# guanlongzhao/fac-via-ppg

Hardware: AMD Instinct MI355X
Metric: 22.05 kHz audio samples/sec end-to-end PPG→wav; real-time factor at batch=1 (higher is better)
Workload: dtype f32

## Files before the change

### fac-via-ppg_amd/csrc/facppg_wg.hip

```cpp
#include <algorithm>
#include <cmath>
#include <cstdlib>
#include <cstring>
#include <new>
#include <type_traits>
#include <vector>

#include "facppg_gemm.h"
#include "facppg_wg_internal.h"

namespace facppg {

thread_local char g_err[512] = "";
void set_error(const char* fmt, ...) {
  va_list ap;
  va_start(ap, fmt);
  vsnprintf(g_err, sizeof(g_err), fmt, ap);
  va_end(ap);
}

namespace {

constexpr int TN = 64;
constexpr int HALO = 128;
// ... 216 lines not shown
      const int mid = (lo + hi + 1) >> 1;
      if (off[mid] <= g) lo = mid; else hi = mid - 1;
    }
    const int q = 4 * (g - off[lo]);
    e = make_int4(lo, q, t_valid[lo] - q, 0);
  }
  table[g] = e;
}

struct WnArgs {
  const float* h_in;
  float* h_out;
  const float* spect;
  float* skip;
  const float4* w1;
  const float* b1;
  const float4* w2;
  const float* b2;
  const int* t_valid;
  int T, hop8, Lp, Lr, dil, first;
  float* save_ts;
  const float* melp;
  const float4* wc;
  int P, Tr, Tqp, ntq, nt, nch, ngc, kc, xcd_map;
  int hop, ksize;
  int flat_cols;
  const int4* groups;
  const float* xa;
  const float* we;
  const float* endb;
  int nconv;
  const float4* seed;
  int seed_nt;
};

typedef float f4u __attribute__((ext_vector_type(4), aligned(4)));

template <int NRB>
__device__ __forceinline__ void load_a(float4 (&a)[4], const float4* __restrict__ p, int rb_stride, int g) {
#pragma unroll
  for (int rb = 0; rb < NRB; ++rb) a[rb] = p[rb * rb_stride + g * 64];
}

template <int NCB, bool K4 = false>
__device__ __forceinline__ void load_b(float (&bv)[4][NCB], const float* lb, int g) {
  if constexpr (K4) {
#pragma unroll
    for (int cb = 0; cb < NCB; ++cb) {
      const float4 v = *reinterpret_cast<const float4*>(lb + ((2 * g) * (32 * NCB) + 32 * cb) * 4);
      bv[0][cb] = v.x; bv[1][cb] = v.y; bv[2][cb] = v.z; bv[3][cb] = v.w;
    }
  } else {
#pragma unroll
    for (int s = 0; s < 4; ++s)
#pragma unroll
      for (int cb = 0; cb < NCB; ++cb) bv[s][cb] = lb[(8 * g + s) * (32 * NCB) + 32 * cb];
  }
}

__device__ __forceinline__ int k4_index(int k, int col, int tnt) { return ((k >> 2) * tnt + col) * 4 + (k & 3); }

template <int NRB, int NCB>
__device__ __forceinline__ void mfma_group(f32x16 (&acc)[4][NCB], const float4 (&a)[4], const float (&bv)[4][NCB]) {
#pragma unroll
  for (int s = 0; s < 4; ++s) {
#pragma unroll
// ... 370 lines not shown
        } else {
          const float vv[4] = {v.x, v.y, v.z, v.w};
          for (int k = 0; k < nv; ++k) gbase[o + k] = vv[k] + (add ? rbase[o + k] : 0.0f);
        }
      }
    }
    return;
  }
#pragma unroll
  for (int rb = 0; rb < NRB2; ++rb) {
    const bool is_res = !LAST && rb < 2;
    const int chb = w * 64 + (rb & 1) * 32 + 4 * kh;
#pragma unroll
    for (int cb = 0; cb < NCB; ++cb) {
      const int col = cb * 32 + li;
      if (col < nvalid) {
#pragma unroll
        for (int r = 0; r < 16; ++r) {
          const int ch = chb + 8 * (r >> 2) + (r & 3);
          if (is_res) {
            const size_t o = ((size_t)b * C + ch) * p.Lp + in_off + col;
            p.h_out[o] = acc[rb][cb][r];
          } else {
            const size_t o = ((size_t)b * C + ch) * p.Lr + sk_off + col;
            p.skip[o] = (p.first ? 0.0f : p.skip[o]) + acc[rb][cb][r];
          }
        }
      }
    }
  }
}

#ifdef FACPPG_WN8_PROF
__device__ unsigned long long g_wn8_prof[12];
#define WN8_STAMP_DECL long long wn8_t = clock64()
#define WN8_STAMP(i)                                                                           \
  do {                                                                                         \
    const long long now__ = clock64();                                                         \
    if (blockIdx.x == 0 && threadIdx.x == 0) { atomicAdd(&g_wn8_prof[i], (unsigned long long)(now__ - wn8_t)); if ((i) == 5) atomicAdd(&g_wn8_prof[6], 1ull); } \
    wn8_t = now__;                                                                             \
  } while (0)
#else
#define WN8_STAMP_DECL
#define WN8_STAMP(i)
#endif

typedef float f32x4s __attribute__((ext_vector_type(4)));
#define FACPPG_AS1 __attribute__((address_space(1)))
typedef float f32x4s __attribute__((ext_vector_type(4)));
__device__ __forceinline__ float4 gld(const float4* q) {
  const f32x4s v = *(const FACPPG_AS1 f32x4s*)q;
  return make_float4(v.x, v.y, v.z, v.w);
}
__device__ __forceinline__ f4u gld(const f4u* q) { return *(const FACPPG_AS1 f4u*)q; }
__device__ __forceinline__ float gld(const float* q) { return *(const FACPPG_AS1 float*)q; }
__device__ __forceinline__ void store_f4(float* g, const float4 v) {
  const f32x4s x = {v.x, v.y, v.z, v.w};
  *(FACPPG_AS1 f32x4s*)g = x;
}
__device__ __forceinline__ void store_f1(float* g, const float v) { *(__attribute__((address_space(1))) float*)g = v; }

template <bool LAST, int NCB, bool EF, bool SEED = false>
__device__ __forceinline__ void wn_layer8_tile(const WnArgs& p, const int lin, float* __restrict__ smem) {
  static_assert(!SEED || NCB == 1, "seeded tiles: 32 frames");
  constexpr int TNt = 32 * NCB;
  WN8_STAMP_DECL;
  const int tid = threadIdx.x, lane = tid & 63, w8 = tid >> 6, wq = w8 >> 1, sub = w8 & 1;
  const int li = lane & 31, kh = lane >> 5;
  const int chb = wq * 64 + sub * 32;
  int b, nvalid, ph, in_off, sk_off, tap0, tap1, tap2, lane_q;
  int tile;
  {
    if (p.xcd_map == 1) { const int r = lin >> 3; ph = (r / p.nt) * 8 + (lin & 7); tile = r % p.nt; }
    else { ph = lin / p.nt; tile = lin % p.nt; }
    if (ph >= p.P) return;
    int qcol;
    if (p.groups) {
      const int4 e = p.groups[tile * (TNt / 4) + lane % (TNt / 4)];
      if (__builtin_amdgcn_readfirstlane(e.z) <= 0) return;
      b = e.x; qcol = e.y; nvalid = e.z;
    } else if (p.flat_cols > 0) {
      const int c0 = tile * TNt + (lane % (TNt / 4)) * 4;
      const int cl = min(c0, p.flat_cols - 4);
      b = cl / p.T; qcol = cl - b * p.T; nvalid = p.flat_cols - c0;
    } else {
      b = tile / p.ntq;
      const int q0 = (tile % p.ntq) * TNt, Tb = p.t_valid ? p.t_valid[b] : p.T;
      if (q0 >= Tb) return;
      qcol = q0 + (lane % (TNt / 4)) * 4; nvalid = Tb - qcol;
    }
    in_off = ph * p.Tqp + HQ + qcol;
    sk_off = ph * p.Tr + qcol;
    lane_q = HQ + qcol;
    {
      const int pm = ph - p.dil, qm = pm >= 0 ? pm / p.P : -((p.P - 1 - pm) / p.P);
      const int pq = ph + p.dil, qp = pq / p.P;
      tap0 = (pm - qm * p.P) * p.Tqp + qm;
      tap1 = ph * p.Tqp;
      tap2 = (pq - qp * p.P) * p.Tqp + qp;
// ... 174 lines not shown
      f32x4 tot = {0.f, 0.f, 0.f, 0.f};
#pragma unroll
      for (int sl = 0; sl < 8; ++sl) {
        const float av[8] = {a0[sl].x, a0[sl].y, a0[sl].z, a0[sl].w, a1[sl].x, a1[sl].y, a1[sl].z, a1[sl].w};
        f32x4 e = {0.f, 0.f, 0.f, 0.f};
#pragma unroll
        for (int g = 0; g < 8; ++g) e = mfma16x16x4(av[g], gb[(8 * sl + g) * TNt * 4], e);
        if (sl == 0) tot = e;
        else { tot[0] += e[0]; tot[1] += e[1]; tot[2] += e[2]; tot[3] += e[3]; }
      }
      if (kq < 2) {
        float* endl = smem + C * TNt + (4 * kq) * TNt + 16 * w8 + pl;
#pragma unroll
        for (int r = 0; r < 4; ++r) endl[r * TNt] = tot[r];
      }
    }
  }
  __syncthreads();
  WN8_STAMP(4);
  if constexpr (EF) {
    const int row = w8 * RPL4 + srow4;
    if (row < 8 && nvalid > 0) {
      float4 v4 = *reinterpret_cast<const float4*>(smem + C * TNt + row * TNt + scol4);
      if constexpr (ESPLIT) {
#pragma unroll
        for (int sl = 1; sl < 8; ++sl) {
          const float4 x = *reinterpret_cast<const float4*>(smem + C * TNt + (sl * 8 + row) * TNt + scol4);
          v4.x += x.x; v4.y += x.y; v4.z += x.z; v4.w += x.w;
        }
      }
      float* g = p.skip + ((size_t)b * 8 + row) * p.Lr + sk_off;
      const float bias = p.endb[row];
      const float vv[4] = {v4.x, v4.y, v4.z, v4.w};
      if (nvalid >= 4) {
        float4 x = make_float4(bias, bias, bias, bias);
        if (!p.first) x = *reinterpret_cast<const float4*>(g);
        store_f4(g, make_float4(x.x + vv[0], x.y + vv[1], x.z + vv[2], x.w + vv[3]));
      } else {
        for (int k = 0; k < nvalid; ++k) store_f1(g + k, (p.first ? bias : g[k]) + vv[k]);
      }
    }
  }
  float* slab = smem + w8 * (32 * TNt);
#pragma unroll
  for (int half = 0; half < NRB2; ++half) {
    const bool is_res = EF || (!LAST && half == 0);
#pragma unroll
    for (int cb = 0; cb < NCB; ++cb)
#pragma unroll
      for (int r = 0; r < 16; ++r) slab[(8 * (r >> 2) + (r & 3) + 4 * kh) * TNt + cb * 32 + li] = acc[half][cb][r];
    const int nv = nvalid;
    if (nv <= 0) continue;
    float* gbase = is_res ? p.h_out + (size_t)b * C * p.Lp + in_off : p.skip + (size_t)b * C * p.Lr + sk_off;
    const float* rbase = is_res ? p.h_in + (size_t)b * C * p.Lp + in_off : gbase;
    const int pitch = is_res ? p.Lp : p.Lr;
    const bool add = is_res || !p.first;
#pragma unroll
    for (int i = 0; i < 32 / RPL4; ++i) {
      const int row = i * RPL4 + srow4;
      const size_t o = (size_t)(chb + row) * pitch;
      float4 v = *reinterpret_cast<const float4*>(slab + row * TNt + scol4);
      if (nv >= 4) {
        if (add) {
          float4 x;
          if (HPRE && is_res) x = hpre[i];
          else x = gld(reinterpret_cast<const float4*>(rbase + o));
          v.x += x.x; v.y += x.y; v.z += x.z; v.w += x.w;
        }
        store_f4(gbase + o, v);
      } else {
        const float vv[4] = {v.x, v.y, v.z, v.w};
        for (int k = 0; k < nv; ++k) store_f1(gbase + o + k, vv[k] + (add ? gld(rbase + o + k) : 0.0f));
      }
    }
  }
// ... 144 lines not shown
#pragma unroll
            for (int cb = 0; cb < NCB; ++cb) acc[rb][cb] = mfma32x32x2(av, bq[s4][cb], acc[rb][cb]);
          }
      }
    }
#pragma unroll
    for (int cb = 0; cb < NCB; ++cb) {
      const int tile = p.tile0 + blk * NCB + cb;
      if (tile >= p.seed_nt) continue;
      float4* dst = p.seeds + (((((size_t)l * p.P + ph) * p.seed_nt + tile) * 8 + w8) * 8) * 64 + lane;
#pragma unroll
      for (int rb = 0; rb < 2; ++rb)
#pragma unroll
        for (int q = 0; q < 4; ++q) {
          const f32x4s x = {acc[rb][cb][4 * q + 0], acc[rb][cb][4 * q + 1], acc[rb][cb][4 * q + 2], acc[rb][cb][4 * q + 3]};
          if constexpr (NT) __builtin_nontemporal_store(x, (FACPPG_AS1 f32x4s*)(dst + (rb * 4 + q) * 64));
          else *(FACPPG_AS1 f32x4s*)(dst + (rb * 4 + q) * 64) = x;
        }
    }
  }
  __syncthreads();
  if (p.counter) {
    if (tid == 0) reinterpret_cast<int*>(smem)[0] = (int)gridDim.x + atomicAdd(p.counter, 1);
    __syncthreads();
    lin = reinterpret_cast<const int*>(smem)[0];
    __syncthreads();
  } else lin += (int)gridDim.x;
  }
}

constexpr int TN16 = 16;

template <bool LAST, bool EF>
__device__ __forceinline__ void wn_layer16_tile(const WnArgs& p, const int ph, const int b, const int q0, float* __restrict__ smem) {
  const int tid = threadIdx.x, lane = tid & 63, w8 = tid >> 6;
  const int pl = lane & 15, kq = lane >> 4;
  const int chb = w8 * 32;
  const int nvalid = (p.t_valid ? p.t_valid[b] : p.T) - q0;
  if (nvalid <= 0) return;
  const int in_off = ph * p.Tqp + HQ + q0, sk_off = ph * p.Tr + q0;
  int tapo[3];
#pragma unroll
  for (int tp = 0; tp < 3; ++tp) {
    const int pp = ph + (tp - 1) * p.dil;
    const int qsh = pp >= 0 ? pp / p.P : -((p.P - 1 - pp) / p.P);
    tapo[tp] = (pp - qsh * p.P) * p.Tqp + HQ + q0 + qsh;
  }
  f32x4 acc[4];
  const float4* wave_a = p.w1 + (w8 * 4) * 64 + lane;
  const float4* wave_c = p.wc + (size_t)ph * (p.ngc / 2) * 2048 + (w8 * 4) * 64 + lane;
  const int nch = pm_chunks(p, ph), ncc = nch - p.nconv, NGC16 = ncc * 4;
  const int srow = tid >> 3, scol = (tid & 7) * 2;
  const bool folded_first = EF && p.nconv == 1;
  const float* hb = (folded_first ? p.xa + (size_t)b * 8 * p.Lp : p.h_in + (size_t)b * C * p.Lp) + scol;
  const float* sb = p.melp + (size_t)b * NMEL * p.Tqp + HQ + q0 + scol;
  typedef float f2u __attribute__((ext_vector_type(2), aligned(4)));
  float2 stg;
  auto stage_load = [&](int c) __attribute__((always_inline)) {
    const bool conv = c >= ncc;
    const int cc = c - ncc;
    const int r = min(c * 64 + srow, p.kc - 1);
    const int j = r / NMEL, m = r - j * NMEL;
    const int tp = folded_first ? min(srow >> 3, 2) : cc >> 2;
    const int chn = folded_first ? (srow & 7) : (cc & 3) * 64 + srow;
    const float* src = conv ? hb + (size_t)chn * p.Lp + (tp == 0 ? tapo[0] : tp == 1 ? tapo[1] : tapo[2])
                            : sb + m * p.Tqp - j;
    const f2u v = *reinterpret_cast<const f2u*>(src);
    stg = make_float2(v.x, v.y);
  };
  const int sw_r = srow & 15, sw_base = (((srow >> 4) * 4 + 2 * (sw_r & 1) + ((sw_r >> 2) & 1)) * TN16) * 4 + 2 * (sw_r >> 3) + ((sw_r >> 1) & 1);
  auto stage_write = [&](int buf) __attribute__((always_inline)) {
    float* dst = smem + buf * (KCH * TN16) + sw_base + scol * 4;
    dst[0] = stg.x; dst[4] = stg.y;
  };
  auto load_a = [&](float4 (&a)[4], int gg) __attribute__((always_inline)) {
    const float4* src = gg < NGC16 ? wave_c + (size_t)gg * 2048 : wave_a + (size_t)(gg - NGC16) * 2048;
#pragma unroll
    for (int rbl = 0; rbl < 4; ++rbl) a[rbl] = src[rbl * 64];
  };
  constexpr int RING = 4;
  float4 ar[RING][4];
  stage_load(0);
#pragma unroll
  for (int i = 0; i < RING - 1; ++i) load_a(ar[i], i);
#pragma unroll
  for (int rbl = 0; rbl < 4; ++rbl) {
    const float4 bv = *reinterpret_cast<const float4*>(p.b1 + (rbl >> 1) * C + chb + (rbl & 1) * 16 + 4 * kq);
    acc[rbl][0] = bv.x; acc[rbl][1] = bv.y; acc[rbl][2] = bv.z; acc[rbl][3] = bv.w;
  }
  stage_write(0);
  __syncthreads();
  for (int c = 0; c < nch; ++c) {
    stage_load(c + 1 < nch ? c + 1 : c);
    const float* lb = smem + (c & 1) * (KCH * TN16) + (kq * TN16 + pl) * 4;
#pragma unroll
    for (int g = 0; g < 4; ++g) {
      load_a(ar[(g + RING - 1) % RING], c * 4 + g + RING - 1);
      __builtin_amdgcn_sched_barrier(0);
      const float4 b4 = *reinterpret_cast<const float4*>(lb + g * (4 * TN16 * 4));
      const float bq[4] = {b4.x, b4.y, b4.z, b4.w};
#pragma unroll
      for (int s = 0; s < 4; ++s)
#pragma unroll
        for (int rbl = 0; rbl < 4; ++rbl) {
          const float4& a4 = ar[g % RING][rbl];
          acc[rbl] = mfma16x16x4(s == 0 ? a4.x : s == 1 ? a4.y : s == 2 ? a4.z : a4.w, bq[s], acc[rbl]);
        }
    }
    stage_write((c + 1) & 1);
    __syncthreads();
  }
#pragma unroll
  for (int rbl = 0; rbl < 2; ++rbl)
#pragma unroll
    for (int r = 0; r < 4; ++r)
      smem[(((2 * w8 + rbl) * 4 + 2 * (r & 1) + (kq & 1)) * TN16 + pl) * 4 + 2 * (kq >> 1) + ((r >> 1) & 1)] = gate_tanh_sigmoid(acc[rbl][r], acc[rbl + 2][r]);
  __syncthreads();
  constexpr int NB2 = EF ? (LAST ? 0 : 2) : LAST ? 2 : 4;
  constexpr bool ROWS256 = LAST || EF;
  float4 hpre[2];
  if constexpr (!LAST) {
    if (nvalid - (lane & 3) * 4 >= 4) {
#pragma unroll
      for (int it = 0; it < 2; ++it)
        hpre[it] = *reinterpret_cast<const float4*>(p.h_in + ((size_t)b * C + chb + it * 16 + (lane >> 2)) * p.Lp + in_off + (lane & 3) * 4);
    }
  }
#pragma unroll
  for (int rbl = 0; rbl < NB2; ++rbl) {
    const float4 bv = *reinterpret_cast<const float4*>(p.b2 + (ROWS256 ? 0 : (rbl >> 1) * C) + chb + (rbl & 1) * 16 + 4 * kq);
    acc[rbl][0] = bv.x; acc[rbl][1] = bv.y; acc[rbl][2] = bv.z; acc[rbl][3] = bv.w;
  }
  if constexpr (NB2 > 0) {
    const float4* ap2 = p.w2 + (w8 * NB2) * 64 + lane;
    const float* lb = smem + (kq * TN16 + pl) * 4;
    auto load_a2 = [&](float4 (&a)[4], int g) __attribute__((always_inline)) {
#pragma unroll
      for (int rbl = 0; rbl < NB2; ++rbl) a[rbl] = ap2[(size_t)g * (NB2 * 8 * 64) + rbl * 64];
    };
#pragma unroll
    for (int i = 0; i < RING - 1; ++i) load_a2(ar[i], i);
    for (int c = 0; c < C / 64; ++c) {
#pragma unroll
      for (int g = 0; g < 4; ++g) {
        load_a2(ar[(g + RING - 1) % RING], c * 4 + g + RING - 1);
        __builtin_amdgcn_sched_barrier(0);
        const float4 b4 = *reinterpret_cast<const float4*>(lb + (4 * c + g) * (4 * TN16 * 4));
        const float bq[4] = {b4.x, b4.y, b4.z, b4.w};
#pragma unroll
        for (int s = 0; s < 4; ++s)
#pragma unroll
          for (int rbl = 0; rbl < NB2; ++rbl) {
            const float4& a4 = ar[g % RING][rbl];
            acc[rbl] = mfma16x16x4(s == 0 ? a4.x : s == 1 ? a4.y : s == 2 ? a4.z : a4.w, bq[s], acc[rbl]);
          }
      }
    }
  }
  if constexpr (EF) {
    const float4* wimg = reinterpret_cast<const float4*>(p.we) + w8 * 128 + lane * 2;
    const float4 a0 = wimg[0], a1 = wimg[1];
    const float av[8] = {a0.x, a0.y, a0.z, a0.w, a1.x, a1.y, a1.z, a1.w};
    f32x4 e = {0.f, 0.f, 0.f, 0.f};
#pragma unroll
    for (int g = 0; g < 8; ++g)
      e = mfma16x16x4(av[g], smem[(((2 * w8 + (g >> 2)) * 4 + 2 * (kq & 1) + (g & 1)) * TN16 + pl) * 4 + 2 * ((g & 3) >> 1) + (kq >> 1)], e);
    if (kq < 2) {
      float* part = smem + C * TN16 + (w8 * 8 + 4 * kq) * TN16 + pl;
#pragma unroll
      for (int r = 0; r < 4; ++r) part[r * TN16] = e[r];
    }
  }
  __syncthreads();
  if constexpr (EF) {
    if (tid < 32) {
      const int row = tid >> 2, c4 = (tid & 3) * 4, nv = nvalid - c4;
      if (nv > 0) {
        const float* part = smem + C * TN16 + row * TN16 + c4;
        float4 t = *reinterpret_cast<const float4*>(part);
#pragma unroll
        for (int sl = 1; sl < 8; ++sl) {
          const float4 x = *reinterpret_cast<const float4*>(part + sl * 8 * TN16);
          t.x += x.x; t.y += x.y; t.z += x.z; t.w += x.w;
        }
        float* g = p.skip + ((size_t)b * 8 + row) * p.Lr + sk_off + c4;
        const float bias = p.endb[row];
        const float vv[4] = {t.x, t.y, t.z, t.w};
        if (nv >= 4) {
          float4 x = make_float4(bias, bias, bias, bias);
          if (!p.first) x = *reinterpret_cast<const float4*>(g);
          *reinterpret_cast<float4*>(g) = make_float4(x.x + vv[0], x.y + vv[1], x.z + vv[2], x.w + vv[3]);
        } else {
          for (int k = 0; k < nv; ++k) g[k] = (p.first ? bias : g[k]) + vv[k];
        }
      }
    }
  }
  float* slab = smem + w8 * (32 * TN16);
  const int erow = lane >> 2, ecol = (lane & 3) * 4;
#pragma unroll
  for (int half = 0; half < NB2 / 2; ++half) {
    const bool is_res = EF || (!LAST && half == 0);
#pragma unroll
    for (int rbl = 0; rbl < 2; ++rbl)
#pragma unroll
      for (int r = 0; r < 4; ++r) slab[(16 * rbl + 4 * kq + r) * TN16 + pl] = acc[half * 2 + rbl][r];
    const int nv = nvalid - ecol;
    if (nv <= 0) continue;
    float* gbase = is_res ? p.h_out + (size_t)b * C * p.Lp + in_off + ecol : p.skip + (size_t)b * C * p.Lr + sk_off + ecol;
    const float* rbase = is_res ? p.h_in + (size_t)b * C * p.Lp + in_off + ecol : gbase;
    const int pitch = is_res ? p.Lp : p.Lr;
    const bool add = is_res || !p.first;
#pragma unroll
    for (int it = 0; it < 2; ++it) {
      const int row = it * 16 + erow;
      const size_t o = (size_t)(chb + row) * pitch;
      float4 v = *reinterpret_cast<const float4*>(slab + row * TN16 + ecol);
      if (nv >= 4) {
        if (add) {
          float4 x;
          if (!LAST && is_res) x = hpre[it];
          else x = *reinterpret_cast<const float4*>(rbase + o);
          v.x += x.x; v.y += x.y; v.z += x.z; v.w += x.w;
        }
        *reinterpret_cast<float4*>(gbase + o) = v;
      } else {
        const float vv[4] = {v.x, v.y, v.z, v.w};
        for (int k = 0; k < nv; ++k) gbase[o + k] = vv[k] + (add ? rbase[o + k] : 0.0f);
      }
    }
  }
}

template <bool LAST, bool EF = false>
__global__ __launch_bounds__(512, 4) void k_wn_layer16(WnArgs p) {
  extern __shared__ __attribute__((aligned(16))) float smem[];
  int ph, tile;
  {
    const int lin = blockIdx.x;
    if (p.xcd_map == 1) { const int r = lin >> 3; ph = (r / p.nt) * 8 + (lin & 7); tile = r % p.nt; }
    else { ph = lin / p.nt; tile = lin % p.nt; }
    if (ph >= p.P) return;
  }
  wn_layer16_tile<LAST, EF>(p, ph, tile / p.ntq, (tile % p.ntq) * TN16, smem);
}

template <bool LAST>
__global__ __launch_bounds__(512, 4) void k_wn_layer_mixed(WnArgs p32, WnArgs p16, int n32) {
  extern __shared__ __attribute__((aligned(16))) float smem[];
  const int lin = (int)blockIdx.x, nt = p32.nt;
  int ph, tile;
  if (p32.xcd_map == 1) { const int r = lin >> 3; ph = (r / nt) * 8 + (lin & 7); tile = r % nt; }
  else { ph = lin / nt; tile = lin % nt; }
  if (ph >= p32.P) return;
  if (tile < n32) wn_layer8_tile<LAST, 1, true, true>(p32, lin, smem);
  else wn_layer16_tile<LAST, true>(p16, ph, 0, 32 * n32 + (tile - n32) * TN16, smem);
}

constexpr int UP_QB = 32;
constexpr int UP_MAXJ = 8;

__global__ __launch_bounds__(256) void k_upsample(const float* __restrict__ mel, const float* __restrict__ W,
                                                  const float* __restrict__ bias, float* __restrict__ spect,
                                                  const int* __restrict__ t_valid, int T, int n_mel, int hop,
                                                  int ksize, int Lr, int n_limit) {
  extern __shared__ float smel[];
  const int b = blockIdx.z, m = blockIdx.y, q0 = blockIdx.x * UP_QB;
  const int Tb = t_valid ? t_valid[b] : T;
  if (q0 >= Tb) return;
  const int nj = (ksize + hop - 1) / hop;
  const int SW = UP_QB + UP_MAXJ;
  for (int i = threadIdx.x; i < n_mel * SW; i += blockDim.x) {
    const int mp = i / SW, tt = i % SW;
    const int t = q0 - (UP_MAXJ - 1) + tt;
    smel[i] = (t >= 0 && t < Tb && tt < UP_QB + UP_MAXJ - 1) ? mel[((size_t)b * n_mel + mp) * T + t] : 0.0f;
  }
  __syncthreads();
  for (int pp = threadIdx.x; pp < hop; pp += blockDim.x) {
    float acc[UP_QB];
    const float bv = bias[m];
#pragma unroll
    for (int q = 0; q < UP_QB; ++q) acc[q] = bv;
    for (int j = 0; j < nj; ++j) {
      const int k = pp + j * hop;
      if (k < ksize) {
        for (int mp = 0; mp < n_mel; ++mp) {
          const float wv = W[((size_t)mp * n_mel + m) * ksize + k];
          const float* sm = smel + mp * SW + (UP_MAXJ - 1) - j;
#pragma unroll
// ... 736 lines not shown
PmLayout pm_layout(const facppg_wg_config& c, int B, int T) {
  PmLayout w;
  w.P = c.hop_length / 8;
  w.L = T * w.P;
  w.La = round_up(w.L, TN);
  w.Tr = round_up(T, TN);
  w.Tqp = HQ + w.Tr + HQ;
  size_t off = 0;
  auto take = [&](size_t floats) { size_t o = off; off += (floats * 4 + 255) / 256 * 256; return o; };
  w.h0 = take((size_t)B * C * w.P * w.Tqp);
  w.h1 = take((size_t)B * C * w.P * w.Tqp);
  w.xa = take((size_t)B * 8 * w.P * w.Tqp);
  w.skip = take((size_t)B * C * w.P * w.Tr);
  w.melp = take((size_t)B * NMEL * w.Tqp);
  w.aud0 = take((size_t)B * 8 * w.La);
  w.aud1 = take((size_t)B * 8 * w.La);
  w.z = take((size_t)B * 8 * w.L + 4);
  w.ngroups = round_up(B * ((T + 3) / 4), 32);
  w.goff = take((size_t)B + 1);
  w.gtab = take((size_t)w.ngroups * 4);
  w.total = off;
  return w;
}
}

extern "C" size_t facppg_wg_workspace_bytes(const facppg_wg* h, int B, int T) {
  if (!h || B <= 0 || T <= 0) return 0;
  if (h->w16) return wg16_workspace_bytes(h, B, T);
  const size_t a = ws_layout(h->cfg, B, T).total, b = pm_layout(h->cfg, B, T).total, c = wgp_workspace_bytes(h, B, T);
  return std::max(a, std::max(b, c));
}

#ifdef FACPPG_WN8_PROF
extern "C" int facppg_debug_wn8_prof(unsigned long long* out12, int reset) {
  FACPPG_HIP_CHECK(hipMemcpyFromSymbol(out12, HIP_SYMBOL(g_wn8_prof), 12 * sizeof(unsigned long long)));
  if (reset) {
    unsigned long long z[12] = {0, 0, 0, 0, 0, 0, 0, 0, 0, 0, 0, 0};
    FACPPG_HIP_CHECK(hipMemcpyToSymbol(HIP_SYMBOL(g_wn8_prof), z, sizeof(z)));
  }
  return FACPPG_OK;
}
#endif

extern "C" int facppg_wg_set_profiling(facppg_wg* h, int enable) {
  WG_REQUIRE_FP32(h, "facppg_wg_set_profiling");
  FACPPG_REQUIRE(h && enable >= 0, FACPPG_EINVAL, "handle is NULL or enable < 0");
  h->profiling = enable;
  h->ev_used = 0;
  if (enable > 1) {
    FACPPG_HIP_CHECK(hipSetDevice(h->device));
    const size_t need = (size_t)enable * 2 * h->cfg.n_flows * h->cfg.wn_layers;
    while (h->ev.size() < need) {
      hipEvent_t ev;
      FACPPG_HIP_CHECK(hipEventCreate(&ev));
      h->ev.push_back(ev);
    }
  }
  return FACPPG_OK;
}

extern "C" int facppg_wg_last_layer_ms(facppg_wg* h, float* avg_ms, int* n_launches) {
  WG_REQUIRE_FP32(h, "facppg_wg_last_layer_ms");
  FACPPG_REQUIRE(h && avg_ms && n_launches, FACPPG_EINVAL, "NULL argument");
  double tot = 0;
  for (int i = 0; i + 1 < h->ev_used; i += 2) {
    float ms = 0;
    FACPPG_HIP_CHECK(hipEventSynchronize(h->ev[i + 1]));
    FACPPG_HIP_CHECK(hipEventElapsedTime(&ms, h->ev[i], h->ev[i + 1]));
    tot += ms;
  }
  *n_launches = h->ev_used / 2 * std::max(1, h->ev_layers);
// ... 110 lines not shown
    FACPPG_REQUIRE(B == 1 && !T_valid_dev && fold, FACPPG_EUNSUPPORTED, "seeded inference: one utterance, folded flow edges");
    FACPPG_REQUIRE(seeded_frames % 32 == 0 && seeded_frames > 0, FACPPG_EUNSUPPORTED,
                   "seeded inference: %d seeded frames, expected a positive multiple of 32", seeded_frames);
    tn = 32;
  }
  const int n32 = seeds && seeded_frames < T ? seeded_frames / 32 : 0;
  const int n16 = n32 ? (T - seeded_frames + TN16 - 1) / TN16 : 0;
  const bool tile16 = tn == TN16, narrow = tn == 32, wide128 = tn == 128;
  WnArgs a;
  memset(&a, 0, sizeof(a));
  a.melp = melp; a.skip = skip; a.t_valid = T_valid_dev; a.T = T; a.hop8 = w.P; a.Lp = w.P * w.Tqp; a.Lr = w.P * w.Tr;
  a.P = w.P; a.Tr = w.Tr; a.Tqp = w.Tqp; a.ntq = (T + tn - 1) / tn; a.nt = a.ntq * B;
  const char* no_flat = getenv("FACPPG_WN_NO_FLAT");
  if (!T_valid_dev && T % 4 == 0 && !no_flat && !tile16) { a.flat_cols = B * T; a.nt = (B * T + tn - 1) / tn; }
  if (T_valid_dev && B > 1 && !no_flat && !tile16) {
    int* goff = (int*)(ws + w.goff);
    int4* gtab = (int4*)(ws + w.gtab);
    k_group_offsets<<<1, 1024, 0, s>>>(T_valid_dev, B, goff);
    k_group_table<<<(w.ngroups + 255) / 256, 256, 0, s>>>(T_valid_dev, goff, B, gtab, w.ngroups);
    a.groups = gtab; a.nt = w.ngroups * 4 / tn;
  }
  a.ngc = h->kcp / 8; a.kc = h->kc; a.hop = c.hop_length; a.ksize = c.upsample_kernel;
  a.xa = xa;
  const char* no_xcd = getenv("FACPPG_WN_NO_XCD_MAP");
  a.xcd_map = ((w.P % 8 == 0) && !no_xcd) ? 1 : 0;
  if (n32) a.nt = n32 + n16;
  const unsigned lgrid = (unsigned)(w.P * a.nt);
  const char* w8env = getenv("FACPPG_WN_8W");
  const int w8mode = seeds ? 1 : w8env ? atoi(w8env) : 1;
  a.seed_nt = w.Tr / 32;
  h->last_tile = tn; h->last_tiles = (int)lgrid;
  h->last_waves = (wide128 || tile16 || (narrow && w8mode != 0) || (!narrow && w8mode == 2)) ? 8 : 4;
  h->ev_layers = c.wn_layers;
  for (int k = nf - 1; k >= 0; --k) {
    if (flow_events && flow_events[k]) FACPPG_HIP_CHECK(hipStreamWaitEvent(s, (hipEvent_t)flow_events[k], 0));
    for (int i = 0; i < c.wn_layers; ++i) {
      a.h_in = hbuf[hi]; a.h_out = hbuf[hi ^ 1];
      a.w1 = h->w1pm[k][i]; a.wc = h->wcpm[k][i]; a.b1 = h->b1pm[k][i]; a.w2 = h->w2[k][i]; a.b2 = h->b2[k][i];
      if (tile16) { a.w1 = h->w1_16[k][i]; a.wc = h->wc_16[k][i]; a.w2 = h->w2_16[k][i]; }
      a.dil = 1 << i; a.first = (i == 0);
      const bool last = i == c.wn_layers - 1;
      a.nconv = NCHH;
      if (fold) {
        a.we = h->we[k][i]; a.endb = h->endb[k];
        a.w2 = tile16 ? h->w2r_16[k][i] : h->w2r[k][i];
        if (i == 0) { a.nconv = 1; a.w1 = tile16 ? h->w1f_16[k] : h->w1f[k]; }
      }
      a.nch = a.nconv + h->kcp / KCH;
      if (h->profiling && i == 0) FACPPG_HIP_CHECK(hipEventRecord(h->ev[h->ev_used++], s));
#define WN_LAUNCH(KERNEL_LAST, KERNEL_MID, THREADS, LDS)              \
  do {                                                                 \
    if (last) KERNEL_LAST<<<lgrid, THREADS, LDS, s>>>(a);              \
    else KERNEL_MID<<<lgrid, THREADS, LDS, s>>>(a);                    \
  } while (0)
      if (fold) {
        if (wide128) WN_LAUNCH((k_wn_layer8<true, 4, true>), (k_wn_layer8<false, 4, true>), 512, 131072 + 4096);
        else if (tile16) WN_LAUNCH((k_wn_layer16<true, true>), (k_wn_layer16<false, true>), 512, 16384 + 4096);
        else if (narrow) {
          if (seeds) {
            a.seed = seeds + (size_t)(k * c.wn_layers + i) * w.P * a.seed_nt * 8 * 8 * 64;
            if (n32) {
              WnArgs a16 = a;
              a16.w1 = i == 0 ? h->w1f_16[k] : h->w1_16[k][i]; a16.wc = h->wc_16[k][i]; a16.w2 = last ? h->w2_16[k][i] : h->w2r_16[k][i];
              a16.flat_cols = 0; a16.groups = nullptr;
              if (last) k_wn_layer_mixed<true><<<lgrid, 512, 32768 + 8 * 1024, s>>>(a, a16, n32);
              else k_wn_layer_mixed<false><<<lgrid, 512, 32768 + 8 * 1024, s>>>(a, a16, n32);
            } else WN_LAUNCH((k_wn_layer8<true, 1, true, true>), (k_wn_layer8<false, 1, true, true>), 512, 32768 + 8 * 1024);
          } else if (w8mode == 0) WN_LAUNCH((k_wn_layer<true, 1, false, true, true>), (k_wn_layer<false, 1, false, true, true>), 256, 32768 + 1024);
          else WN_LAUNCH((k_wn_layer8<true, 1, true>), (k_wn_layer8<false, 1, true>), 512, 32768 + 8 * 1024);
        } else if (w8mode == 2) WN_LAUNCH((k_wn_layer8<true, 2, true>), (k_wn_layer8<false, 2, true>), 512, 65536 + 2048);
        else WN_LAUNCH((k_wn_layer<true, 2, false, true, true>), (k_wn_layer<false, 2, false, true, true>), 256, 65536 + 2048);
      } else {
        if (tile16) WN_LAUNCH((k_wn_layer16<true>), (k_wn_layer16<false>), 512, 16384);
        else if (narrow) {
          if (w8mode == 0) WN_LAUNCH((k_wn_layer<true, 1, false, true>), (k_wn_layer<false, 1, false, true>), 256, 32768);
          else WN_LAUNCH((k_wn_layer8<true, 1>), (k_wn_layer8<false, 1>), 512, 32768);
        } else if (w8mode == 2) WN_LAUNCH((k_wn_layer8<true, 2>), (k_wn_layer8<false, 2>), 512, 65536);
        else WN_LAUNCH((k_wn_layer<true, 2, false, true>), (k_wn_layer<false, 2, false, true>), 256, 65536);
      }
#undef WN_LAUNCH
      if (!last) hi ^= 1;
      if (h->profiling && last) FACPPG_HIP_CHECK(hipEventRecord(h->ev[h->ev_used++], s));
    }
    e.aud_in = aud[ai]; e.aud_out = aud[ai ^ 1]; e.h_out = hbuf[hi];
    e.end_w = h->end_w[k]; e.end_b = h->end_b[k]; e.winv = h->winv[k];
    e.final_flow = (k == 0);
    e.swap = c.alternate_halves && (k & 1);
    e.swap_next = c.alternate_halves && k > 0 && ((k - 1) & 1);
    e.z_early = nullptr;
    if (h->early[k]) { e.z_early = z + z_off; z_off += (size_t)B * c.n_early_size * w.L; }
    if (k > 0) { e.start_w = h->start_w[k - 1]; e.start_b = h->start_b[k - 1]; }
    const int cn = 2 * h->n_half[k] + (h->early[k] ? 2 : 0);
    if (k > 0) FACPPG_REQUIRE(cn == 2 * h->n_half[k - 1], FACPPG_EUNSUPPORTED, "flow %d channel mismatch", k);
    else FACPPG_REQUIRE(cn == 8, FACPPG_EUNSUPPORTED, "final flow must yield n_group channels");
    switch (h->n_half[k]) {
      case 1: launch_flow_end<1>(h->early[k], fqs, fgrid, s, e); break;
      case 2: launch_flow_end<2>(h->early[k], fqs, fgrid, s, e); break;
      case 3: launch_flow_end<3>(h->early[k], fqs, fgrid, s, e); break;
      case 4: launch_flow_end<4>(h->early[k], fqs, fgrid, s, e); break;
      default: FACPPG_REQUIRE(false, FACPPG_EUNSUPPORTED, "n_half %d", h->n_half[k]);
    }
    ai ^= 1;
  }
  FACPPG_HIP_CHECK(hipGetLastError());
  return FACPPG_OK;
}

extern "C" int facppg_wg_infer(facppg_wg* h, const float* mel_dev, const int32_t* T_valid_dev, const float* z_dev,
                               uint64_t seed, float sigma, int B, int T, float* audio_dev, void* ws_, size_t ws_bytes,
                               void* stream_) {
  WG_REQUIRE_FP32(h, "facppg_wg_infer");
  FACPPG_REQUIRE(h && mel_dev && audio_dev && ws_, FACPPG_EINVAL, "NULL argument");
  FACPPG_REQUIRE(B > 0 && T > 0, FACPPG_EINVAL, "B and T must be positive (got %d, %d)", B, T);
  const facppg_wg_config& c = h->cfg;
  const WsLayout w = ws_layout(c, B, T);
  {
    const size_t need = facppg_wg_workspace_bytes(h, B, T);
    FACPPG_REQUIRE(ws_bytes >= need, FACPPG_EWORKSPACE, "workspace has %zu bytes, need %zu", ws_bytes, need);
  }
  FACPPG_REQUIRE(B <= 65535, FACPPG_EINVAL, "B too large");
  {
    int tot = h->n_rem[c.n_flows - 1];
    for (int k = 0; k < c.n_flows; ++k) tot += h->early[k] ? c.n_early_size : 0;
    FACPPG_REQUIRE(tot == 8, FACPPG_EUNSUPPORTED, "noise channel count %d != n_group", tot);
  }
  const char* unfolded = getenv("FACPPG_WG_UNFOLDED");
  if (!unfolded || atoi(unfolded) == 0)
// ... 547 lines not shown
```

Baseline: 4.405 million.

## Fuse WaveGlow flow-end coupling and next start conv into last WN layer

```diff
diff --git a/fac-via-ppg_amd/csrc/facppg_wg.hip b/fac-via-ppg_amd/csrc/facppg_wg.hip
--- a/fac-via-ppg_amd/csrc/facppg_wg.hip
+++ b/fac-via-ppg_amd/csrc/facppg_wg.hip
@@ -272,6 +272,15 @@
   int nconv;
   const float4* seed;
   int seed_nt;
+  int fe_mode, fe_swap, fe_swap_next, fe_L, fe_La;
+  float fe_sigma;
+  const float* fe_aud_in;
+  float* fe_aud_out;
+  const float* fe_z_early;
+  const float* fe_winv;
+  const float* fe_start_w;
+  const float* fe_start_b;
+  float* fe_xa_out;
 };
 
 typedef float f4u __attribute__((ext_vector_type(4), aligned(4)));
@@ -708,16 +717,20 @@
 }
 
 #ifdef FACPPG_WN8_PROF
-__device__ unsigned long long g_wn8_prof[12];
-#define WN8_STAMP_DECL long long wn8_t = clock64()
+__device__ unsigned long long g_wn_prof[2][3][8];
+#define WN8_STAMP_DECL(TK, ON, KIND)                                  \
+  long long wn8_t = wall_clock64();                                   \
+  const bool wn8_on = (ON) && threadIdx.x == 0;                       \
+  unsigned long long* const wn8_slot = g_wn_prof[TK][KIND]
 #define WN8_STAMP(i)                                                                           \
   do {                                                                                         \
-    const long long now__ = clock64();                                                         \
-    if (blockIdx.x == 0 && threadIdx.x == 0) { atomicAdd(&g_wn8_prof[i], (unsigned long long)(now__ - wn8_t)); if ((i) == 5) atomicAdd(&g_wn8_prof[6], 1ull); } \
+    if ((i) == 0 || (i) == 5) asm volatile("s_waitcnt vmcnt(0)" ::: "memory");                 \
+    const long long now__ = wall_clock64();                                                    \
+    if (wn8_on) { atomicAdd(&wn8_slot[i], (unsigned long long)(now__ - wn8_t)); if ((i) == 5) atomicAdd(&wn8_slot[7], 1ull); } \
     wn8_t = now__;                                                                             \
   } while (0)
 #else
-#define WN8_STAMP_DECL
+#define WN8_STAMP_DECL(TK, ON, KIND)
 #define WN8_STAMP(i)
 #endif
 
@@ -736,11 +749,98 @@
 }
 __device__ __forceinline__ void store_f1(float* g, const float v) { *(__attribute__((address_space(1))) float*)g = v; }
 
+template <int H, bool EARLY, int TW>
+__device__ __forceinline__ void wn_edge_column(const WnArgs& p, const int ph, const int x, const int col, float* __restrict__ smem) {
+  constexpr int CC = 2 * H, CN = EARLY ? CC + 2 : CC, HN = CN / 2;
+  const int pos = x * p.P + ph;
+  float a[CC], y[CN], o[CC];
+#pragma unroll
+  for (int j = 0; j < CC; ++j) a[j] = gld(p.fe_aud_in + (size_t)j * p.fe_La + pos);
+  if constexpr (EARLY) {
+#pragma unroll
+    for (int j = 0; j < 2; ++j) y[j] = p.fe_sigma * gld(p.fe_z_early + (size_t)j * p.fe_L + pos);
+  }
+#pragma unroll
+  for (int j = 0; j < CC; ++j) o[j] = smem[j * TW + col];
+#pragma unroll
+  for (int j = 0; j < H; ++j) {
+    const float t = ((p.fe_swap ? a[j] : a[H + j]) - o[j]) / expf(o[H + j]);
+    if (p.fe_swap) a[j] = t;
+    else a[H + j] = t;
+  }
+#pragma unroll
+  for (int i = 0; i < CC; ++i) {
+    float v = 0.0f;
+#pragma unroll
+    for (int j = 0; j < CC; ++j) v = fmaf(p.fe_winv[i * CC + j], a[j], v);
+    y[(EARLY ? 2 : 0) + i] = v;
+  }
+#pragma unroll
+  for (int j = 0; j < CN; ++j) store_f1(p.fe_aud_out + (size_t)j * p.fe_La + pos, y[j]);
+  float* xd = p.fe_xa_out + ph * p.Tqp + HQ + x;
+#pragma unroll
+  for (int j = 0; j < 8; ++j) {
+    const float a0 = j < HN ? (p.fe_swap_next ? y[HN + (j < HN ? j : 0)] : y[j < HN ? j : 0]) : j == HN ? 1.0f : 0.0f;
+    store_f1(xd + (size_t)j * p.Lp, a0);
+    if (j < HN) smem[(8 + j) * TW + col] = a0;
+  }
+}
+
+template <int TW>
+__device__ __forceinline__ void wn_edge_tile(const WnArgs& p, const int ph, const int q0, const int ncol, float* __restrict__ smem) {
+  const int tid = threadIdx.x, lane = tid & 63, w8 = tid >> 6;
+  const int hn = (p.fe_mode >> 1) + (p.fe_mode & 1);
+  constexpr int F4 = TW / 4, RP = 64 / F4, NPASS = 32 / RP;
+  const int srow = lane / F4, col4 = (lane % F4) * 4;
+  float sb[NPASS], sw[NPASS][4];
+#pragma unroll
+  for (int i = 0; i < NPASS; ++i) {
+    const int ch = 32 * w8 + i * RP + srow;
+    sb[i] = gld(p.fe_start_b + ch);
+#pragma unroll
+    for (int j = 0; j < 4; ++j) sw[i][j] = j < hn ? gld(p.fe_start_w + ch * hn + j) : 0.0f;
+  }
+  __syncthreads();
+  if (tid < ncol) {
+    const int x = q0 + tid;
+    switch (p.fe_mode) {
+      case 2: wn_edge_column<1, false, TW>(p, ph, x, tid, smem); break;
+      case 3: wn_edge_column<1, true, TW>(p, ph, x, tid, smem); break;
+      case 4: wn_edge_column<2, false, TW>(p, ph, x, tid, smem); break;
+      case 5: wn_edge_column<2, true, TW>(p, ph, x, tid, smem); break;
+      case 6: wn_edge_column<3, false, TW>(p, ph, x, tid, smem); break;
+      case 7: wn_edge_column<3, true, TW>(p, ph, x, tid, smem); break;
+      default: wn_edge_column<4, false, TW>(p, ph, x, tid, smem); break;
+    }
+  }
+  __syncthreads();
+  const int nv = ncol - col4;
+  if (nv <= 0) return;
+  float* hd = p.h_out + ph * p.Tqp + HQ + q0 + col4;
+#pragma unroll
+  for (int i = 0; i < NPASS; ++i) {
+    const int ch = 32 * w8 + i * RP + srow;
+    float v[4] = {sb[i], sb[i], sb[i], sb[i]};
+#pragma unroll
+    for (int j = 0; j < 4; ++j) {
+      if (j < hn) {
+        const float4 a0 = *reinterpret_cast<const float4*>(smem + (8 + j) * TW + col4);
+        v[0] = fmaf(sw[i][j], a0.x, v[0]); v[1] = fmaf(sw[i][j], a0.y, v[1]);
+        v[2] = fmaf(sw[i][j], a0.z, v[2]); v[3] = fmaf(sw[i][j], a0.w, v[3]);
+      }
+    }
+    float* g = hd + (size_t)ch * p.Lp;
+    if (nv >= 4) store_f4(g, make_float4(v[0], v[1], v[2], v[3]));
+    else
+      for (int k = 0; k < nv; ++k) store_f1(g + k, v[k]);
+  }
+}
+
 template <bool LAST, int NCB, bool EF, bool SEED = false>
 __device__ __forceinline__ void wn_layer8_tile(const WnArgs& p, const int lin, float* __restrict__ smem) {
   static_assert(!SEED || NCB == 1, "seeded tiles: 32 frames");
   constexpr int TNt = 32 * NCB;
-  WN8_STAMP_DECL;
+  WN8_STAMP_DECL(0, blockIdx.x == 0, p.first ? 0 : LAST ? 2 : 1);
   const int tid = threadIdx.x, lane = tid & 63, w8 = tid >> 6, wq = w8 >> 1, sub = w8 & 1;
   const int li = lane & 31, kh = lane >> 5;
   const int chb = wq * 64 + sub * 32;
@@ -981,15 +1081,29 @@
       float* g = p.skip + ((size_t)b * 8 + row) * p.Lr + sk_off;
       const float bias = p.endb[row];
       const float vv[4] = {v4.x, v4.y, v4.z, v4.w};
+      float fs[4] = {0.0f, 0.0f, 0.0f, 0.0f};
       if (nvalid >= 4) {
         float4 x = make_float4(bias, bias, bias, bias);
         if (!p.first) x = *reinterpret_cast<const float4*>(g);
-        store_f4(g, make_float4(x.x + vv[0], x.y + vv[1], x.z + vv[2], x.w + vv[3]));
+        fs[0] = x.x + vv[0]; fs[1] = x.y + vv[1]; fs[2] = x.z + vv[2]; fs[3] = x.w + vv[3];
+        store_f4(g, make_float4(fs[0], fs[1], fs[2], fs[3]));
       } else {
-        for (int k = 0; k < nvalid; ++k) store_f1(g + k, (p.first ? bias : g[k]) + vv[k]);
-      }
-    }
-  }
+#pragma unroll
+        for (int k = 0; k < 3; ++k)
+          if (k < nvalid) { fs[k] = (p.first ? bias : g[k]) + vv[k]; store_f1(g + k, fs[k]); }
+      }
+      if constexpr (LAST && ESPLIT) {
+        if (p.fe_mode) *reinterpret_cast<float4*>(smem + row * TNt + scol4) = make_float4(fs[0], fs[1], fs[2], fs[3]);
+      }
+    }
+  }
+  if constexpr (LAST && ESPLIT) {
+    if (p.fe_mode) {
+      const int q0 = (p.flat_cols > 0 ? tile : tile % p.ntq) * TNt;
+      wn_edge_tile<TNt>(p, ph, q0, min(TNt, (p.t_valid ? p.t_valid[0] : p.T) - q0), smem);
+    }
+  }
+  WN8_STAMP(6);
   float* slab = smem + w8 * (32 * TNt);
 #pragma unroll
   for (int half = 0; half < NRB2; ++half) {
@@ -1200,12 +1314,14 @@
 constexpr int TN16 = 16;
 
 template <bool LAST, bool EF>
-__device__ __forceinline__ void wn_layer16_tile(const WnArgs& p, const int ph, const int b, const int q0, float* __restrict__ smem) {
+__device__ __forceinline__ void wn_layer16_tile(const WnArgs& p, const int ph, const int b, const int q0, float* __restrict__ smem,
+                                                const bool stamp = false) {
   const int tid = threadIdx.x, lane = tid & 63, w8 = tid >> 6;
   const int pl = lane & 15, kq = lane >> 4;
   const int chb = w8 * 32;
   const int nvalid = (p.t_valid ? p.t_valid[b] : p.T) - q0;
   if (nvalid <= 0) return;
+  WN8_STAMP_DECL(1, stamp, p.first ? 0 : LAST ? 2 : 1);
   const int in_off = ph * p.Tqp + HQ + q0, sk_off = ph * p.Tr + q0;
   int tapo[3];
 #pragma unroll
@@ -1258,6 +1374,7 @@
   }
   stage_write(0);
   __syncthreads();
+  WN8_STAMP(0);
   for (int c = 0; c < nch; ++c) {
     stage_load(c + 1 < nch ? c + 1 : c);
     const float* lb = smem + (c & 1) * (KCH * TN16) + (kq * TN16 + pl) * 4;
@@ -1278,12 +1395,14 @@
     stage_write((c + 1) & 1);
     __syncthreads();
   }
+  WN8_STAMP(1);
 #pragma unroll
   for (int rbl = 0; rbl < 2; ++rbl)
 #pragma unroll
     for (int r = 0; r < 4; ++r)
       smem[(((2 * w8 + rbl) * 4 + 2 * (r & 1) + (kq & 1)) * TN16 + pl) * 4 + 2 * (kq >> 1) + ((r >> 1) & 1)] = gate_tanh_sigmoid(acc[rbl][r], acc[rbl + 2][r]);
   __syncthreads();
+  WN8_STAMP(2);
   constexpr int NB2 = EF ? (LAST ? 0 : 2) : LAST ? 2 : 4;
   constexpr bool ROWS256 = LAST || EF;
   float4 hpre[2];
@@ -1325,6 +1444,7 @@
       }
     }
   }
+  WN8_STAMP(3);
   if constexpr (EF) {
     const float4* wimg = reinterpret_cast<const float4*>(p.we) + w8 * 128 + lane * 2;
     const float4 a0 = wimg[0], a1 = wimg[1];
@@ -1340,6 +1460,7 @@
     }
   }
   __syncthreads();
+  WN8_STAMP(4);
   if constexpr (EF) {
     if (tid < 32) {
       const int row = tid >> 2, c4 = (tid & 3) * 4, nv = nvalid - c4;
@@ -1354,16 +1475,27 @@
         float* g = p.skip + ((size_t)b * 8 + row) * p.Lr + sk_off + c4;
         const float bias = p.endb[row];
         const float vv[4] = {t.x, t.y, t.z, t.w};
+        float fs[4] = {0.0f, 0.0f, 0.0f, 0.0f};
         if (nv >= 4) {
           float4 x = make_float4(bias, bias, bias, bias);
           if (!p.first) x = *reinterpret_cast<const float4*>(g);
-          *reinterpret_cast<float4*>(g) = make_float4(x.x + vv[0], x.y + vv[1], x.z + vv[2], x.w + vv[3]);
+          fs[0] = x.x + vv[0]; fs[1] = x.y + vv[1]; fs[2] = x.z + vv[2]; fs[3] = x.w + vv[3];
+          store_f4(g, make_float4(fs[0], fs[1], fs[2], fs[3]));
         } else {
-          for (int k = 0; k < nv; ++k) g[k] = (p.first ? bias : g[k]) + vv[k];
+#pragma unroll
+          for (int k = 0; k < 3; ++k)
+            if (k < nv) { fs[k] = (p.first ? bias : g[k]) + vv[k]; g[k] = fs[k]; }
         }
-      }
-    }
-  }
+        if constexpr (LAST) {
+          if (p.fe_mode) *reinterpret_cast<float4*>(smem + row * TN16 + c4) = make_float4(fs[0], fs[1], fs[2], fs[3]);
+        }
+      }
+    }
+    if constexpr (LAST) {
+      if (p.fe_mode) wn_edge_tile<TN16>(p, ph, q0, min(TN16, nvalid), smem);
+    }
+  }
+  WN8_STAMP(6);
   float* slab = smem + w8 * (32 * TN16);
   const int erow = lane >> 2, ecol = (lane & 3) * 4;
 #pragma unroll
@@ -1391,13 +1523,14 @@
           else x = *reinterpret_cast<const float4*>(rbase + o);
           v.x += x.x; v.y += x.y; v.z += x.z; v.w += x.w;
         }
-        *reinterpret_cast<float4*>(gbase + o) = v;
+        store_f4(gbase + o, v);
       } else {
         const float vv[4] = {v.x, v.y, v.z, v.w};
         for (int k = 0; k < nv; ++k) gbase[o + k] = vv[k] + (add ? rbase[o + k] : 0.0f);
       }
     }
   }
+  WN8_STAMP(5);
 }
 
 template <bool LAST, bool EF = false>
@@ -1410,7 +1543,7 @@
     else { ph = lin / p.nt; tile = lin % p.nt; }
     if (ph >= p.P) return;
   }
-  wn_layer16_tile<LAST, EF>(p, ph, tile / p.ntq, (tile % p.ntq) * TN16, smem);
+  wn_layer16_tile<LAST, EF>(p, ph, tile / p.ntq, (tile % p.ntq) * TN16, smem, ph == 0 && tile == 0);
 }
 
 template <bool LAST>
@@ -1422,7 +1555,7 @@
   else { ph = lin / nt; tile = lin % nt; }
   if (ph >= p32.P) return;
   if (tile < n32) wn_layer8_tile<LAST, 1, true, true>(p32, lin, smem);
-  else wn_layer16_tile<LAST, true>(p16, ph, 0, 32 * n32 + (tile - n32) * TN16, smem);
+  else wn_layer16_tile<LAST, true>(p16, ph, 0, 32 * n32 + (tile - n32) * TN16, smem, ph == 0 && tile == n32);
 }
 
 constexpr int UP_QB = 32;
@@ -2225,11 +2358,12 @@
 }
 
 #ifdef FACPPG_WN8_PROF
-extern "C" int facppg_debug_wn8_prof(unsigned long long* out12, int reset) {
-  FACPPG_HIP_CHECK(hipMemcpyFromSymbol(out12, HIP_SYMBOL(g_wn8_prof), 12 * sizeof(unsigned long long)));
+extern "C" int facppg_debug_wn_prof(unsigned long long* out48, int reset) {
+  FACPPG_HIP_CHECK(hipMemcpyFromSymbol(out48, HIP_SYMBOL(g_wn_prof), 48 * sizeof(unsigned long long)));
   if (reset) {
-    unsigned long long z[12] = {0, 0, 0, 0, 0, 0, 0, 0, 0, 0, 0, 0};
-    FACPPG_HIP_CHECK(hipMemcpyToSymbol(HIP_SYMBOL(g_wn8_prof), z, sizeof(z)));
+    unsigned long long z[48];
+    memset(z, 0, sizeof(z));
+    FACPPG_HIP_CHECK(hipMemcpyToSymbol(HIP_SYMBOL(g_wn_prof), z, sizeof(z)));
   }
   return FACPPG_OK;
 }
@@ -2406,10 +2540,32 @@
   h->last_tile = tn; h->last_tiles = (int)lgrid;
   h->last_waves = (wide128 || tile16 || (narrow && w8mode != 0) || (!narrow && w8mode == 2)) ? 8 : 4;
   h->ev_layers = c.wn_layers;
+  const char* fuse_env = getenv("FACPPG_WG_EDGE_FUSE");
+  const bool fuse = fold && fqs && B == 1 && (tile16 || (narrow && w8mode != 0)) && (!fuse_env || atoi(fuse_env) != 0);
   for (int k = nf - 1; k >= 0; --k) {
     if (flow_events && flow_events[k]) FACPPG_HIP_CHECK(hipStreamWaitEvent(s, (hipEvent_t)flow_events[k], 0));
+    e.aud_in = aud[ai]; e.aud_out = aud[ai ^ 1];
+    e.end_w = h->end_w[k]; e.end_b = h->end_b[k]; e.winv = h->winv[k];
+    e.final_flow = (k == 0);
+    e.swap = c.alternate_halves && (k & 1);
+    e.swap_next = c.alternate_halves && k > 0 && ((k - 1) & 1);
+    e.z_early = nullptr;
+    if (h->early[k]) { e.z_early = z + z_off; z_off += (size_t)B * c.n_early_size * w.L; }
+    if (k > 0) { e.start_w = h->start_w[k - 1]; e.start_b = h->start_b[k - 1]; }
+    const int cn = 2 * h->n_half[k] + (h->early[k] ? 2 : 0);
+    if (k > 0) FACPPG_REQUIRE(cn == 2 * h->n_half[k - 1], FACPPG_EUNSUPPORTED, "flow %d channel mismatch", k);
+    else FACPPG_REQUIRE(cn == 8, FACPPG_EUNSUPPORTED, "final flow must yield n_group channels");
+    FACPPG_REQUIRE(h->n_half[k] >= 1 && h->n_half[k] <= 4, FACPPG_EUNSUPPORTED, "n_half %d", h->n_half[k]);
+    const bool fuse_k = fuse && k > 0;
     for (int i = 0; i < c.wn_layers; ++i) {
       a.h_in = hbuf[hi]; a.h_out = hbuf[hi ^ 1];
+      a.fe_mode = 0;
+      if (fuse_k && i == c.wn_layers - 1) {
+        a.fe_mode = 2 * h->n_half[k] + (h->early[k] ? 1 : 0);
+        a.fe_swap = e.swap; a.fe_swap_next = e.swap_next; a.fe_L = w.L; a.fe_La = w.La; a.fe_sigma = sigma;
+        a.fe_aud_in = e.aud_in; a.fe_aud_out = e.aud_out; a.fe_z_early = e.z_early; a.fe_winv = e.winv;
+        a.fe_start_w = e.start_w; a.fe_start_b = e.start_b; a.fe_xa_out = xa;
+      }
       a.w1 = h->w1pm[k][i]; a.wc = h->wcpm[k][i]; a.b1 = h->b1pm[k][i]; a.w2 = h->w2[k][i]; a.b2 = h->b2[k][i];
       if (tile16) { a.w1 = h->w1_16[k][i]; a.wc = h->wc_16[k][i]; a.w2 = h->w2_16[k][i]; }
       a.dil = 1 << i; a.first = (i == 0);
@@ -2456,17 +2612,11 @@
       if (!last) hi ^= 1;
       if (h->profiling && last) FACPPG_HIP_CHECK(hipEventRecord(h->ev[h->ev_used++], s));
     }
-    e.aud_in = aud[ai]; e.aud_out = aud[ai ^ 1]; e.h_out = hbuf[hi];
-    e.end_w = h->end_w[k]; e.end_b = h->end_b[k]; e.winv = h->winv[k];
-    e.final_flow = (k == 0);
-    e.swap = c.alternate_halves && (k & 1);
-    e.swap_next = c.alternate_halves && k > 0 && ((k - 1) & 1);
-    e.z_early = nullptr;
-    if (h->early[k]) { e.z_early = z + z_off; z_off += (size_t)B * c.n_early_size * w.L; }
-    if (k > 0) { e.start_w = h->start_w[k - 1]; e.start_b = h->start_b[k - 1]; }
-    const int cn = 2 * h->n_half[k] + (h->early[k] ? 2 : 0);
-    if (k > 0) FACPPG_REQUIRE(cn == 2 * h->n_half[k - 1], FACPPG_EUNSUPPORTED, "flow %d channel mismatch", k);
-    else FACPPG_REQUIRE(cn == 8, FACPPG_EUNSUPPORTED, "final flow must yield n_group channels");
+    if (fuse_k) {
+      hi ^= 1; ai ^= 1;
+      continue;
+    }
+    e.h_out = hbuf[hi];
     switch (h->n_half[k]) {
       case 1: launch_flow_end<1>(h->early[k], fqs, fgrid, s, e); break;
       case 2: launch_flow_end<2>(h->early[k], fqs, fgrid, s, e); break;
```

New measurement: 4.500 million (median of 6 runs). +2.2%, better.
